# seqan/lambda

Measured on AMD Instinct MI355X. Metric: GCUPS (gapped extension, full-rectangle parity mode; pass-1 cells per second of whole step) searchp BLOSUM62, higher is better.
Workload: dtype f16x2 (exact small integers) + int32

## Files before the change

### lambda_amd/csrc/lx_ckpt.hip

```cpp
#include <hip/hip_runtime.h>

#include <algorithm>
#include <cstdlib>

#include "lx_aids.h"
#include "lx_dp_common.h"

namespace lx
{

#ifndef LX_CKPT_EVERY
#define LX_CKPT_EVERY 16
#endif
constexpr int kCkptEvery = LX_CKPT_EVERY;
#ifndef LX_CKPT_UNROLL
#define LX_CKPT_UNROLL 4
#endif
#define LX_CKPT_PRAGMA(x) _Pragma(#x)
#define LX_CKPT_UNROLL_N(n) LX_CKPT_PRAGMA(unroll n)
#define LX_CKPT_UNROLL_PRAGMA LX_CKPT_UNROLL_N(LX_CKPT_UNROLL)
#ifndef LX_BT_TILE_AT
#define LX_BT_TILE_AT 40
#endif
#ifndef LX_BT_WAVES
#define LX_BT_WAVES 2
#endif
#ifndef LX_BT_HOPS
#define LX_BT_HOPS 2
#endif
#ifndef LX_BT_REFILL_AT
#define LX_BT_REFILL_AT 12
#endif
#ifndef LX_CKPT_FWD_WAVES
#define LX_CKPT_FWD_WAVES 4
#endif

template <int G>
__host__ __device__ constexpr uint32_t bnd_quad_index(uint32_t quad, uint32_t g)
{
    return quad * G + g;
}
#ifndef LX_CKPT_ROWCK_LANE_MAJOR
#define LX_CKPT_ROWCK_LANE_MAJOR 1
#endif
template <int G, int kCkDw>
__host__ __device__ constexpr uint32_t rowck_quad_index(uint32_t m, uint32_t g, uint32_t x)
{
    return LX_CKPT_ROWCK_LANE_MAJOR ? (m * G + g) * (kCkDw / 4) + x : (m * (kCkDw / 4) + x) * G + g;
}
template <int G, int C>
struct CkptLayout
{
    static constexpr int kCkDw = (C + 3) / 4 * 4;
    __host__ __device__ static constexpr uint64_t bnd_dwords(uint32_t steps_cap) { return (uint64_t)steps_cap * G; }
    __host__ __device__ static constexpr uint64_t slot_dwords(uint32_t steps_cap)
    {
        return bnd_dwords(steps_cap) + (uint64_t)(steps_cap / kCkptEvery) * G * kCkDw;
    }
};

__device__ __forceinline__ uint32_t pack16(int lo, int hi)
{
    return ((uint32_t)lo & 0xffffu) | ((uint32_t)hi << 16);
}

template <int G, int C, bool KNOWN, bool MULTI>
__global__ __launch_bounds__(64, (KNOWN ? LX_CKPT_FWD_WAVES : 3)) void ckpt_forward_kernel(TraceParams p)
{
    using Geo = ScoreGeo<G, C>;
    using Lay = CkptLayout<G, C>;
    extern __shared__ uint32_t lds[];

    int const  lane     = threadIdx.x;
    int const  grp      = lane / G;
    int const  g        = lane % G;
    bool const is_first = (g == 0);
    bool const is_last  = (g == G - 1);

    uint64_t const e     = (uint64_t)blockIdx.x * Geo::kGroups + grp;
    uint64_t       limit = p.n;
    if (p.count_ptr)
    {
        uint64_t const total = *p.count_ptr;
        limit = total > p.chunk_start ? min(p.n, total - p.chunk_start) : 0;
        if ((uint64_t)blockIdx.x * Geo::kGroups >= limit)
            return;
    }
    bool active = e < limit;
    if (active && p.src && p.src[e] == 0xffffffffu)
        active = false;
    bool in_list = e < limit;
    if constexpr (!KNOWN)
    {
        if (p.fixup)
        {
            bool const mine = in_list && p.score_out[e] == -1;
            if (__ballot(mine) == 0)
                return;
            active  = active && mine;
            in_list = mine;
        }
    }

    ScoringDev const * __restrict__ sc = p.sc;
    int const      ge    = sc->ge;
    int const      g2    = sc->g2;
    int const      nrows = p.nrows;
    uint32_t const padt  = (uint32_t)(nrows - 1);

    int             lq = 0, ls = 0;
    uint8_t const * q = p.q_res;
    uint8_t const * s = p.s_res;
    uint64_t        q_off = 0;
    if (e < limit)
    {
        Extension const x = p.ext[e];
        lq    = (int)x.q_len;
        q_off = x.q_off;
        q += x.q_off;
        if (active)
        {
            ls = (int)x.s_len;
            if (ls != 0)
                s += x.s_off;
        }
    }
    int const share  = p.shared_profile > 1 ? min(p.shared_profile, Geo::kGroups) : 1;
    int const leader = (grp / share) * share * G;
    if (share > 1)
    {
        uint32_t const qlo = (uint32_t)__shfl((int)(uint32_t)q_off, leader), qhi = (uint32_t)__shfl((int)(q_off >> 32), leader);
        int const      l0  = __shfl(lq, leader);
        bool const     lead_in = __shfl(in_list ? 1 : 0, leader) != 0;
        if (in_list && lead_in && (q_off != (((uint64_t)qhi << 32) | qlo) || lq != l0))
            atomicExch(p.err, 2);
    }

    int       ls_max    = ls;
    int       npanels   = (lq + Geo::kPanel - 1) / Geo::kPanel;
    int const my_panels = npanels;
#pragma unroll
    for (int off = 32; off >= 1; off >>= 1)
    {
        ls_max = max(ls_max, __shfl_xor(ls_max, off));
        if constexpr (MULTI)
            npanels = max(npanels, __shfl_xor(npanels, off));
    }
    ls_max = __builtin_amdgcn_readfirstlane(ls_max);
    if constexpr (MULTI)
        npanels = max(1, __builtin_amdgcn_readfirstlane(npanels));
    else
        npanels = 1;

    bool bad = false;
    if (active && (lq > (MULTI ? (int)p.panels_cap : 1) * Geo::kPanel || (uint32_t)((ls + G - 1 + 3) & ~3) > p.steps_cap || ls > 65535))
    {
        bad = true;
        atomicExch(p.err, 3);
    }
    if (bad)
        ls = 0;

    int32_t * carry = nullptr;
    if constexpr (MULTI)
    {
        if (npanels > 1)
        {
            uint32_t base = 0;
            int      ok   = 1;
            if (is_first && my_panels > 1 && active && !bad)
            {
                base = atomicAdd(p.ws_top, (uint32_t)ls);
                if (base + (uint32_t)ls > p.ws_cap)
                {
                    ok = 0;
                    atomicExch(p.err, 1);
                }
            }
#pragma unroll
            for (int off = G / 2; off >= 1; off >>= 1)
            {
                base = max(base, (uint32_t)__shfl_xor((int)base, off));
                ok   = min(ok, __shfl_xor(ok, off));
            }
            if (my_panels > 1 && ok)
                carry = p.ws + 2ull * base;
            else if (my_panels > 1)
            {
                bad = true;
                ls  = 0;
            }
        }
    }

    int const      slot_dw     = (grp / share) * (nrows * Geo::kRowDw);
    uint32_t const row_base_dw = (uint32_t)(slot_dw + g);
    int const      steps       = (ls_max + G - 1 + 3) & ~3;
    uint32_t const lsc         = (uint32_t)max(ls, 1) - 1u;

    uint32_t * slot = p.trace + e * p.slot_stride;
    uint32_t   ovf_tag = 0;
    if constexpr (!KNOWN)
    {
        if (p.fixup && p.ovf_count)
        {
            uint32_t idx = 0;
            if (is_first && active && !bad)
                idx = atomicAdd(p.ovf_count, 1u);
            idx = (uint32_t)__shfl((int)idx, grp * G);
            if (active && !bad && idx >= p.ovf_cap)
            {
                bad = true;
                ls  = 0;
                atomicExch(p.err, 4);
            }
            ovf_tag = idx + 1;
            slot    = p.ovf + (uint64_t)(bad ? 0 : idx) * p.ovf_stride;
        }
    }
    int tgt = 0;
    if constexpr (KNOWN)
        tgt = active ? p.score_in[e] : 0;
    int kcol = 0x7fffffff, krow = 0;
    int run_best = 0, run_strip = 0, run_row = 0, run_tie = 0;
    uint64_t const panel_dw = Lay::slot_dwords(p.steps_cap);

    for (int panel = 0; panel < npanels; ++panel)
    {
    bool const    in_panel = panel < my_panels;
    bool const    store_ok = active && !bad && in_panel;
    uint32_t * const pslot = slot + (uint64_t)(MULTI ? panel : 0) * panel_dw;
    uint4 * const rowck    = reinterpret_cast<uint4 *>(pslot + Lay::bnd_dwords(p.steps_cap));
    int lbest = 0, lrow = 0, ltie = 0;
    bool use_carry_in = false, do_carry_out = false;
    if constexpr (MULTI)
    {
        use_carry_in = is_first && panel > 0 && in_panel && carry != nullptr;
        do_carry_out = is_last && panel + 1 < my_panels && carry != nullptr;
    }

    int const col0 = (MULTI ? panel * Geo::kPanel : 0) + g * C;
    build_profile<G, C>(lds, slot_dw, g, q, lq, col0, sc->mat_adj, nrows, grp % share == 0);
    __builtin_amdgcn_fence(__ATOMIC_RELEASE, "wavefront");
    __builtin_amdgcn_wave_barrier();

    int z = ge * g;
    int Hrow[C], F0[C];
#pragma unroll
    for (int c = 0; c < C; ++c)
    {
        Hrow[c] = z + ge;
        F0[c]   = z;
    }
    int diag0 = z + ge;
    int sendH = z + ge;
    int sendE = kNegInf;
    int g2v = g2, gev = ge;
    LX_OPAQUE(g2v);
    LX_OPAQUE(gev);

    uint32_t * const stage = lds + ((Geo::kGroups + share - 1) / share) * (nrows * Geo::kRowDw) + lane * 4;
    uint4 * const    bnd   = reinterpret_cast<uint4 *>(pslot);

    auto step = [&](int k, uint32_t t)
    {
        int const        i    = k - g;
        uint32_t const * prow = lds + (row_base_dw + t * (uint32_t)Geo::kRowDw);
        uint32_t         pw[Geo::kD];
#pragma unroll
        for (int d = 0; d < Geo::kD; ++d)
            pw[d] = prow[d * G];

        int bndH = z, bndE = kNegInf;
        if constexpr (MULTI)
        {
            if (use_carry_in && (unsigned)i < (unsigned)ls)
            {
                bndH = carry[2 * i];
                bndE = carry[2 * i + 1];
            }
        }
        int const recvH = shift_from_left<G>(sendH, bndH, is_first);
        int       Ecur  = shift_from_left<G>(sendE, bndE, is_first);
        int       dg    = diag0;
        diag0           = recvH;

        int const zn     = z - gev;
        int       rowmax = z;
        int       h      = 0;
#pragma unroll
        for (int c = 0; c < C; ++c)
        {
            int const sub = (int)(int8_t)(pw[c >> 2] >> (8 * (c & 3)));
            int const tt  = dg + sub;
            dg            = Hrow[c];
            h             = max3i(tt, Ecur, F0[c]);
            LX_OPAQUE(h);
            int const A   = h + g2v;
            F0[c]         = max3i(F0[c], A, zn);
            LX_OPAQUE(F0[c]);
            Ecur          = max(Ecur, A) + gev;
            if (c & 1)
                rowmax = max3i(rowmax, Hrow[c - 1], h);
            else if (c == C - 1)
                rowmax = max(rowmax, h);
            Hrow[c] = h;
        }
        if constexpr (KNOWN)
        {
            if (tgt > 0 && rowmax == tgt + z && (unsigned)i < (unsigned)ls)
            {
#pragma unroll
                for (int c = C - 1; c >= 0; --c)
                    if (Hrow[c] == rowmax && col0 + c < kcol)
                    {
                        kcol = col0 + c;
                        krow = i;
                    }
            }
        }
        else
        {
            int const  cand = rowmax - z;
            bool const gt   = cand > lbest;
            ltie            = gt ? 0 : (ltie | (cand == lbest ? 1 : 0));
            lrow            = gt ? i : lrow;
            lbest           = max(lbest, cand);
        }
        sendH = h;
        sendE = Ecur;
        if constexpr (MULTI)
        {
            if (do_carry_out && (unsigned)i < (unsigned)ls)
            {
                carry[2 * i]     = sendH;
                carry[2 * i + 1] = sendE;
            }
        }
        stage[k & 3] = pack16(h - z, max(Ecur - z, -32768));
        z            = zn;
    };
    auto checkpoint = [&](int k)
    {
        if (!store_ok)
            return;
#pragma unroll
        for (int x = 0; x < Lay::kCkDw / 4; ++x)
        {
            uint32_t w[4];
#pragma unroll
            for (int b = 0; b < 4; ++b)
            {
                int const c = 4 * x + b;
                w[b]        = c < C ? pack16(Hrow[c < C ? c : 0] - (z + gev), F0[c < C ? c : 0] - z) : 0u;
            }
            rowck[rowck_quad_index<G, Lay::kCkDw>((uint32_t)(k / kCkptEvery), (uint32_t)g, (uint32_t)x)] = make_uint4(w[0], w[1], w[2], w[3]);
        }
    };

    auto fetch_checked = [&](int k0, uint32_t (&t)[4])
    {
#pragma unroll
        for (int u = 0; u < 4; ++u)
        {
            uint32_t const i   = (uint32_t)(k0 + u - g);
            uint32_t const idx = min(i, lsc);
            t[u]               = s[idx];
        }
    };
    auto mask_checked = [&](int k0, uint32_t (&t)[4])
    {
#pragma unroll
        for (int u = 0; u < 4; ++u)
        {
            uint32_t const i = (uint32_t)(k0 + u - g);
            t[u]             = (i < (uint32_t)ls) ? (t[u] & (kAlph - 1)) : padt;
        }
    };

    uint32_t tn[4];
    fetch_checked(0, tn);
    for (int k0 = 0; k0 < steps; k0 += 4)
    {
        uint32_t tc[4] = {tn[0], tn[1], tn[2], tn[3]};
        mask_checked(k0, tc);
        fetch_checked(k0 + 4, tn);
        uint32_t const tcp = tc[0] | (tc[1] << 8) | (tc[2] << 16) | (tc[3] << 24);
LX_CKPT_UNROLL_PRAGMA
        for (int u = 0; u < 4; ++u)
            step(k0 + u, (tcp >> (8 * u)) & 0xffu);
        if (store_ok)
            bnd[bnd_quad_index<G>((uint32_t)k0 / 4, (uint32_t)g)] = *reinterpret_cast<uint4 const *>(stage);
        if (((k0 + 3) % kCkptEvery) == kCkptEvery - 1)
            checkpoint(k0 + 3);
    }

    if constexpr (!KNOWN)
    {
        int gbest = lbest, gstrip = g, grow = lrow, gtie = ltie;
#pragma unroll
        for (int off = 1; off < G; off <<= 1)
        {
            int const  ob = __shfl_xor(gbest, off), os = __shfl_xor(gstrip, off), orow = __shfl_xor(grow, off), ot = __shfl_xor(gtie, off);
            bool const take = ob > gbest || (ob == gbest && os < gstrip);
            gbest  = take ? ob : gbest;
            gstrip = take ? os : gstrip;
            grow   = take ? orow : grow;
            gtie   = take ? ot : gtie;
        }
        bool const take = gbest > run_best;
        run_best  = take ? gbest : run_best;
        run_strip = take ? (MULTI ? panel * G : 0) + gstrip : run_strip;
        run_row   = take ? grow : run_row;
        run_tie   = take ? gtie : run_tie;
    }
    if constexpr (MULTI)
    {
        if (npanels > 1)
        {
            __builtin_amdgcn_fence(__ATOMIC_RELEASE, "workgroup");
            __builtin_amdgcn_s_waitcnt(0);
            __builtin_amdgcn_fence(__ATOMIC_ACQUIRE, "workgroup");
        }
    }
    __builtin_amdgcn_wave_barrier();
    }

    if constexpr (KNOWN)
    {
#pragma unroll
        for (int off = 1; off < G; off <<= 1)
        {
            int const  oc = __shfl_xor(kcol, off), orow = __shfl_xor(krow, off);
            bool const take = oc < kcol;
            kcol = take ? oc : kcol;
            krow = take ? orow : krow;
        }
        if (in_list && is_first)
        {
            EndCell ec{};
            if (bad || (tgt > 0 && kcol == 0x7fffffff))
                ec.score = -1;
            else if (tgt > 0)
            {
                ec.score = tgt;
                ec.q_end = kcol + 1;
                ec.s_end = krow + 1;
            }
            p.ends[e] = ec;
        }
    }
    else
    {
        int const gbest = run_best, gstrip = run_strip, grow = run_row, gtie = run_tie;
        if (in_list && is_first)
        {
            EndCell ec{};
            if (bad)
                ec.score = -1;
            else if (active && gbest > 0)
            {
                ec.score = gbest;
                ec.q_end = -(gstrip + 1);
                ec.s_end = grow + 1;
                ec.flags = (gtie ? kEndAmbiguous : 0) | (int32_t)(ovf_tag << kEndOverflowShift);
            }
            p.ends[e] = ec;
            if (p.score_out)
                p.score_out[e] = bad ? -1 : (active ? gbest : 0);
        }
    }
}

template <int G, int C>
__global__ __launch_bounds__(64, LX_BT_WAVES) void ckpt_backtrace_kernel(TraceParams p)
{
    using Lay               = CkptLayout<G, C>;
    using L16               = Ckpt16Layout<G, C>;
    constexpr int kNibDw    = (C + 7) / 8;
    constexpr int kFar      = -(1 << 28);
    static_assert(kCkptEvery == 16, "the diagonal shortcut reads at most 16 residues per sequence");
    __shared__ int8_t   smat4[kAlph * kAlph];
    __shared__ int8_t   smat1n[kAlph * kAlph];
    __shared__ uint32_t tiles[kCkptEvery * kNibDw * 64];
    for (int x = threadIdx.x; x < kAlph * kAlph; x += blockDim.x)
    {
        int const v = p.sc->mat[x];
        smat4[x]    = (int8_t)((v < -32 || v > 31) ? -125 : 4 * v + 3);
        smat1n[x]   = (int8_t)(x == kAlph * kAlph - 1 ? 0 : min(-v, 127));
    }
    __syncthreads();
    uint32_t const lane  = threadIdx.x;
    uint64_t       limit = p.n;
    if (p.count_ptr)
    {
        uint64_t const total = *p.count_ptr;
        limit = total > p.chunk_start ? min(p.n, total - p.chunk_start) : 0;
    }
    int const ge = p.sc->ge, g2 = p.sc->g2;
    int const ge4 = 4 * p.sc->ge, go4 = 4 * p.sc->go;
    uint64_t panel_dw = Lay::slot_dwords(p.steps_cap), panel16_dw = L16::slot_dwords(p.steps_cap), bnd_dw = Lay::bnd_dwords(p.steps_cap);

    bool             have = false, blocked = false, done = false, need_col = false, scan = false, c16 = false;
    uint64_t         po = 0;
    uint64_t         pos = 0;
    EndCell          ec{};
    uint32_t const * slot = nullptr;
    uint32_t         oct_mul = G, ck_mul = G * (L16::kCkDw / 4);
    uint64_t         ck16_off = 0;
    uint8_t const *  q = nullptr, * s = nullptr;
    uint8_t *        ops_al = nullptr;
    uint32_t         cap = 0, a0 = 0, apos = 0, acc = 0, n = 0;
    int              lq = 0, ls = 0;
    int              i = 0, j = 0, end_i = 0, end_j = 0;
    int              res_col = C, res_row = 0x7fffffff;
    int              nar_cw = C, nar_j0 = 0x7fffffff, nar_st0 = 0x7fffffff;
    auto locate = [&](int aj, int & st, int & j0, int & cw)
    {
        if (aj >= nar_j0)
        {
            int const jl = aj - nar_j0;
            int const gl = nar_cw == (3 * C + 3) / 4 ? jl / ((3 * C + 3) / 4) : nar_cw == (C + 1) / 2 ? jl / ((C + 1) / 2) : jl / ((C + 3) / 4);
            st = nar_st0 + gl;
            j0 = nar_j0 + gl * nar_cw;
            cw = nar_cw;
        }
        else
        {
            st = aj / C;
            j0 = st * C;
            cw = C;
        }
    };
    int              mode = 0;
    int              left = 0;
    int32_t          nm = 0, nx = 0, np = 0, go = 0, gx = 0;
    bool const       rle_mode = p.rle != nullptr;
    uint32_t         run_op = 3, run_len = 0, ncodes = 0;

    auto dec = [](uint32_t bits16) -> int { return (int)(int16_t)bits16; };
    auto expand = [](uint32_t code16) -> uint32_t
    {
        uint32_t const H = code16 & 0x7ffu;
        return H | ((H - (code16 >> 11)) << 16);
    };
    auto bnd_of = [&](uint32_t pn) { return reinterpret_cast<uint4 const *>(slot + (uint64_t)pn * (c16 ? panel16_dw : panel_dw)); };
    auto rowck_of = [&](uint32_t pn)
    {
        return reinterpret_cast<uint4 const *>(slot + (c16 ? (uint64_t)pn * panel16_dw + ck16_off
                                                           : (uint64_t)pn * panel_dw + bnd_dw));
    };
    auto oct16_index = [&](uint32_t o, uint32_t g_) -> uint32_t { return o * oct_mul + g_; };
    auto ck16_index  = [&](uint32_t m_, uint32_t g_, uint32_t x_) -> uint32_t { return m_ * ck_mul + g_ * (L16::kCkDw / 4) + x_; };
    auto rowck_word = [&](uint32_t m, uint32_t st, uint32_t c) -> uint32_t
    {
        if (c16)
            return expand(reinterpret_cast<uint16_t const *>(rowck_of(st / G) + ck16_index(m, st % G, c / 8))[c % 8]);
        return reinterpret_cast<uint32_t const *>(rowck_of(st / G) + rowck_quad_index<G, Lay::kCkDw>(m, st % G, c / 4))[c % 4];
    };
    auto bnd_word_of = [&](uint32_t st, uint32_t k) -> uint32_t
    {
        if (c16)
            return expand(reinterpret_cast<uint16_t const *>(bnd_of(st / G) + oct16_index(k / 8, st % G))[k & 7]);
        return reinterpret_cast<uint32_t const *>(bnd_of(st / G) + bnd_quad_index<G>(k / 4, st % G))[k & 3];
    };
    auto put_byte = [&](uint32_t byte)
    {
        acc |= byte << (8 * (apos & 3));
        if ((apos & 3) == 0)
        {
            if (apos + 3 <= a0 + cap - 1)
                *reinterpret_cast<uint32_t *>(ops_al + apos) = acc;
            else
                for (uint32_t b = 0; b < 4 && apos + b <= a0 + cap - 1; ++b)
                    ops_al[apos + b] = (uint8_t)(acc >> (8 * b));
            acc = 0;
        }
        --apos;
    };
    auto emit = [&](uint32_t op)
    {
        if (rle_mode)
        {
            uint32_t const oc = op == (uint32_t)'M' ? 0u : (op == (uint32_t)'D' ? 1u : 2u);
            if (oc != run_op || run_len == 64)
            {
                if (run_op != 3)
                {
                    put_byte((run_op << 6) | (run_len - 1));
                    ++ncodes;
                }
                run_op  = oc;
                run_len = 0;
            }
            ++run_len;
        }
        else
            put_byte(op);
        ++n;
    };

    auto begin_extension = [&](uint64_t e)
    {
        uint64_t oi = e;
        if (p.src)
        {
            uint32_t const sidx = p.src[e];
            if (sidx == 0xffffffffu)
                return;
            oi = sidx;
        }
        pos                = e;
        po                 = p.out_by_pos ? e : oi;
        uint64_t const  se = p.slot_by_src ? oi : e;
        ec                 = p.ends[se];
        Extension const x  = p.ext[e];
        if (ec.score <= 0)
        {
            Hsp out{};
            out.score     = ec.score < 0 ? -1 : 0;
            p.out_hsp[po] = out;
            return;
        }
        c16                = (ec.flags & kEndCompact) != 0;
        uint32_t const ovf = (uint32_t)ec.flags >> kEndOverflowShift;
        slot               = ovf ? p.ovf + (uint64_t)(ovf - 1) * p.ovf_stride : p.trace + se * p.slot_stride;
        uint32_t steps_e   = p.steps_cap;
        if (p.wf_tab && !ovf)
        {
            WfSlots const  t      = p.wf_tab[se / 16];
            uint64_t const stride = (uint64_t)t.panels_cap * (c16 ? L16::slot_dwords(t.steps_cap) : Lay::slot_dwords(t.steps_cap));
            slot                  = ((p.split_n != 0 && se >= p.split_n) ? p.trace2 : p.trace) + t.off_dw + (se % 16) * stride;
            steps_e               = t.steps_cap;
        }
        panel_dw           = Lay::slot_dwords(steps_e);
        panel16_dw         = L16::slot_dwords(steps_e);
        bnd_dw             = Lay::bnd_dwords(steps_e);
        oct_mul            = G;
        ck_mul             = G * (L16::kCkDw / 4);
        ck16_off           = L16::bnd_dwords(steps_e);
        if (!ovf && (ec.flags & kEndWaveSlots))
        {
            constexpr uint32_t kW = 128 / G;
            uint64_t const     w  = se % kW;
            slot     = p.trace + (se - w) * p.slot_stride + w * (G * 4);
            oct_mul  = kW * G;
            ck_mul   = kW * G * (L16::kCkDw / 4);
            ck16_off = (uint64_t)kW * L16::bnd_dwords(steps_e) - w * (G * 4) + w * (G * L16::kCkDw);
        }
        q                  = p.q_res + x.q_off;
        s                  = p.s_res + x.s_off;
        uint8_t * const ops = p.out_ops + (p.ops_off ? p.ops_off[po] : po * p.ops_stride);
        cap                = x.q_len + x.s_len;
        lq                 = (int)x.q_len;
        ls                 = (int)x.s_len;
        i                  = ec.s_end - 1;
        j                  = ec.q_end - 1;
        {
            int const code = (ec.flags >> kEndNarrowShift) & 3;
            int const last = max(1, (lq + G * C - 1) / (G * C)) - 1;
            nar_cw  = narrow_strip_cols(C, code);
            nar_j0  = code ? last * (G * C) : 0x7fffffff;
            nar_st0 = code ? last * G : 0x7fffffff;
        }
        need_col = ec.q_end < 0;
        if (need_col)
        {
            int const st = -ec.q_end - 1;
            j = st >= nar_st0 ? nar_j0 + (st - nar_st0) * nar_cw + (nar_cw - 1) : st * C + (C - 1);
            scan = (ec.flags & kEndAmbiguous) != 0;
            if (scan)
            {
                int const gl = st % G;
                i            = min(((i + gl) / kCkptEvery) * kCkptEvery - gl + kCkptEvery - 1, ls - 1);
            }
        }
        end_i = i;
        end_j = j;
        res_col = C;
        res_row = 0x7fffffff;
        mode = 0;
        left = ec.score;
        n    = 0;
        nm = nx = np = go = gx = 0;
        a0     = (uint32_t)(reinterpret_cast<uintptr_t>(ops) & 3);
        ops_al = ops - a0;
        apos   = a0 + cap - 1;
        acc    = 0;
        run_op  = 3;
        run_len = 0;
        ncodes  = 0;
        have    = true;
        done    = false;
        blocked = false;
    };

    auto close_ops = [&]()
    {
        if (mode != 0)
            go += 1;
        if (rle_mode && run_op != 3)
        {
            put_byte((run_op << 6) | (run_len - 1));
            ++ncodes;
        }
        if ((apos & 3) != 3)
            for (uint32_t b = (apos & 3) + 1; b < 4 && (apos & ~3u) + b <= a0 + cap - 1; ++b)
                ops_al[(apos & ~3u) + b] = (uint8_t)(acc >> (8 * b));
    };
    auto finish_extension = [&](uint64_t at)
    {
        if (rle_mode && ec.score >= 0)
        {
            if (at + ncodes > p.rle_cap)
            {
                atomicExch(p.err, 5);
                ec.score = -1;
            }
            else
            {
                uint8_t const * const src = ops_al + apos + 1;
                uint8_t * const       dst = p.rle + at;
                for (uint32_t k = 0; k < ncodes; ++k)
                    dst[k] = src[k];
            }
        }
        Hsp out{};
        if (ec.score < 0)
            out.score = -1;
        else
        {
            out.score              = ec.score;
            out.q_begin            = j + 1;
            out.q_end              = end_j + 1;
            out.s_begin            = i + 1;
            out.s_end              = end_i + 1;
            out.n_ops              = (int32_t)n;
            out.num_matches        = nm;
            out.num_mismatches     = nx;
            out.num_positives      = np;
            out.num_gap_opens      = go;
            out.num_gap_extensions = gx;
            out.ops_shift          = rle_mode ? (int32_t)(uint32_t)at : (int32_t)(cap - n);
        }
        p.out_hsp[po] = out;
        if (rle_mode && p.rle_len)
            p.rle_len[pos] = ec.score > 0 ? ncodes : 0u;
        have          = false;
    };


    auto load_diagonal = [&](int ci, int cj, int k, uint32_t (&qw)[4], uint32_t (&sw)[4])
    {
#pragma unroll
        for (int d = 0; d < 4; ++d)
        {
            qw[d] = *reinterpret_cast<unaligned_u32 const *>(q + (cj - k + 1) + 4 * d);
            sw[d] = *reinterpret_cast<unaligned_u32 const *>(s + (ci - k + 1) + 4 * d);
        }
    };
    auto take_diagonal = [&](int k, int Hb, bool verify, uint32_t (&qw)[4], uint32_t (&sw)[4]) -> bool
    {
#pragma unroll
        for (int d = 0; d < 4; ++d)
        {
            int const      nb  = k - 4 * d;
            uint32_t const pad = nb >= 4 ? 0u : (nb <= 0 ? 0x1f1f1f1fu : (0x1f1f1f1fu << (8 * nb)));
            qw[d]              = (qw[d] & 0x1f1f1f1fu) | pad;
            sw[d]              = (sw[d] & 0x1f1f1f1fu) | pad;
        }
        int      P = 0, cnt = 0;
        uint32_t posbits = 0;
        int32_t  tmb = 0;
        bool const bs = p.bs_match_rule != 0;
#pragma unroll
        for (int u = kCkptEvery - 1; u >= 0; --u)
        {
            int const      d   = u >> 2, b = u & 3;
            uint32_t const idx = (((qw[d] >> (8 * b)) & 0x1fu) << 5) | ((sw[d] >> (8 * b)) & 0x1fu);
            int const      nv  = (int)smat1n[idx];
            bool const     take = P < left;
            int const      nve = take ? nv : 0;
            cnt += take ? 1 : 0;
            P -= nve;
            posbits = __builtin_amdgcn_alignbit(posbits, (uint32_t)nve, 31);
            if (bs)
                tmb += (take && nv == (int)smat1n[(idx >> 5) * (kAlph + 1)]) ? 1 : 0;
        }
        int const beyond = left > 0 ? kCkptEvery - k : 0;
        cnt -= beyond;
        tmb -= bs ? beyond : 0;
        int const  L       = left - P;
        bool const stopped = cnt < k;
        if (!(stopped ? (L == 0) : (!verify || L == Hb)))
            return false;
        int32_t tm = tmb;
        if (!bs)
        {
            int const lo = k - cnt;
#pragma unroll
            for (int d = 0; d < 4; ++d)
            {
                uint32_t const x   = qw[d] ^ sw[d];
                uint32_t const nz  = (x + 0x7f7f7f7fu) & 0x80808080u;
                int const      b0  = max(lo - 4 * d, 0), b1 = min(k - 4 * d, 4);
                uint32_t const msk = b1 > b0 ? ((b1 >= 4 ? 0xffffffffu : ((1u << (8 * b1)) - 1u)) & ~((1u << (8 * b0)) - 1u)) : 0u;
                tm += __popc(~nz & 0x80808080u & msk);
            }
        }
        left = L;
        nm += tm;
        nx += cnt - tm;
        np += __popc(posbits);
        if (rle_mode)
        {
            int left_m = cnt;
            while (left_m > 0)
            {
                if (run_op != 0 || run_len == 64)
                {
                    if (run_op != 3)
                    {
                        put_byte((run_op << 6) | (run_len - 1));
                        ++ncodes;
                    }
                    run_op  = 0;
                    run_len = 0;
                }
                int const take = min(left_m, 64 - (int)run_len);
                run_len += (uint32_t)take;
                left_m -= take;
            }
        }
        else if (cnt > 0)
        {
            uint32_t const hi = apos, lo = apos + 1 - (uint32_t)cnt, Dtop = hi & ~3u, Dlow = lo & ~3u;
#pragma unroll
            for (int sl = 0; sl < 5; ++sl)
            {
                uint32_t const D = Dtop - 4u * sl;
                if (Dtop >= 4u * sl && D >= Dlow)
                {
                    uint32_t const b0  = lo > D ? lo - D : 0, b1 = sl == 0 ? hi - D : 3u;
                    uint32_t const msk = (b1 >= 3 ? 0xffffffffu : ((1u << (8 * (b1 + 1))) - 1u)) & ~((1u << (8 * b0)) - 1u);
                    uint32_t const val = (sl == 0 ? acc : 0u) | (0x4d4d4d4du & msk);
                    if (lo <= D)
                    {
                        if (sl != 0 || D + 3 <= a0 + cap - 1)
                            *reinterpret_cast<uint32_t *>(ops_al + D) = val;
                        else
                            for (uint32_t bb = 0; bb < 4 && D + bb <= a0 + cap - 1; ++bb)
                                ops_al[D + bb] = (uint8_t)(val >> (8 * bb));
                        acc = 0;
                    }
                    else
                        acc = val;
                }
            }
            apos -= (uint32_t)cnt;
        }
        n += (uint32_t)cnt;
        i -= cnt;
        j -= cnt;
        done = stopped;
        return true;
    };

    bool queue_empty = false;
    int const tile_at = p.bt_tile_at > 0 ? p.bt_tile_at : LX_BT_TILE_AT, refill_at = p.bt_refill_at > 0 ? p.bt_refill_at : LX_BT_REFILL_AT;
    for (;;)
    {
        bool fin       = have && (done || i < 0 || j < 0 || n >= cap);
        bool can       = have && !fin && !blocked && !need_col && mode == 0;
        bool tile_need = have && !fin && !can;
        int  n_can = __popcll(__ballot(can)), n_tile = __popcll(__ballot(tile_need));
        int const n_idle = 64 - n_can - n_tile;
        bool run_tile = n_can == 0 || n_tile >= tile_at;
        if (n_idle > 0 && (run_tile || n_idle >= refill_at))
        {
            if (fin)
                close_ops();
            uint64_t at = 0;
            if (rle_mode)
            {
                uint32_t const mine = fin ? ncodes : 0u;
                uint32_t       incl = mine;
#pragma unroll
                for (int off = 1; off < 64; off <<= 1)
                {
                    uint32_t const up = (uint32_t)__shfl_up((int)incl, off);
                    if ((int)lane >= off)
                        incl += up;
                }
                uint32_t const     total = (uint32_t)__shfl((int)incl, 63);
                unsigned long long base  = 0;
                if (lane == 63 && total != 0)
                    base = atomicAdd(p.rle_top, (unsigned long long)total);
                base = ((unsigned long long)(uint32_t)__shfl((int)(base >> 32), 63) << 32) | (uint32_t)__shfl((int)(uint32_t)base, 63);
                at   = base + incl - mine;
            }
            if (fin)
                finish_extension(at);
            if (!queue_empty)
            {
                uint64_t const want = __ballot(!have);
                if (want != 0)
                {
                    uint32_t  base   = 0;
                    int const leader = __ffsll((unsigned long long)want) - 1;
                    if ((int)lane == leader)
                        base = atomicAdd(p.work_counter, (uint32_t)__popcll(want));
                    base = (uint32_t)__shfl((int)base, leader);
                    if ((uint64_t)base + (uint32_t)__popcll(want) >= limit)
                        queue_empty = true;
                    if (!have)
                    {
                        uint64_t const e = (uint64_t)base + (uint32_t)__popcll(want & ((1ull << lane) - 1ull));
                        if (e < limit)
                            begin_extension(e);
                    }
                }
            }
            fin       = have && (done || i < 0 || j < 0 || n >= cap);
            can       = have && !fin && !blocked && !need_col && mode == 0;
            tile_need = have && !fin && !can;
            n_can     = __popcll(__ballot(can));
            n_tile    = __popcll(__ballot(tile_need));
            if (n_can == 0 && n_tile == 0)
            {
                if (__ballot(have) == 0 && queue_empty)
                    break;
                if (__ballot(have) == 0)
                    continue;
            }
            run_tile = n_can == 0 || n_tile >= tile_at;
        }

        if (!run_tile)
        {
            if (can)
            {
                int      hk[LX_BT_HOPS];
                uint32_t hw[LX_BT_HOPS], hqw[LX_BT_HOPS][4], hsw[LX_BT_HOPS][4];
                int      ci = i, cj = j;
#pragma unroll
                for (int h = 0; h < LX_BT_HOPS; ++h)
                {
                    bool const on = ci >= 0 && cj >= 0;
                    int const ai = max(ci, 0), aj = max(cj, 0);
                    int st, j0, cw;
                    locate(aj, st, j0, cw);
                    int const c  = aj - j0;
                    int const gl = st % G;
                    int const m  = (ai + gl) / kCkptEvery;
                    int const r_base = m * kCkptEvery - gl;
                    int const kt = ai - r_base + 1, kl = c + 1;
                    int const k  = min(min(kt, kl), ai + 1);
                    int const bi = ai - k, bj = aj - k;
                    hk[h] = on ? k : 0;
                    hw[h] = 0;
                    if (on && bi >= 0 && bj >= 0)
                        hw[h] = (kl <= kt) ? bnd_word_of((uint32_t)(st - 1), (uint32_t)(bi + (st - 1) % G))
                                           : rowck_word((uint32_t)(m - 1), (uint32_t)st, (uint32_t)(bj - j0));
                    load_diagonal(ai, aj, k, hqw[h], hsw[h]);
                    ci -= k;
                    cj -= k;
                }
#pragma unroll
                for (int h = 0; h < LX_BT_HOPS; ++h)
                    if (hk[h] > 0 && !blocked && !done)
                        if (!take_diagonal(hk[h], dec(hw[h] & 0xffffu), true, hqw[h], hsw[h]))
                            blocked = true;
            }
            continue;
        }

        if (tile_need)
        {
        int st, j0, cw;
        locate(j, st, j0, cw);
        int const pn = st / G, gl = st % G;
        int const m  = (i + gl) / kCkptEvery;
        int const k_base = m * kCkptEvery;
        int const r_base = k_base - gl;
        uint4 const * const rowck = rowck_of((uint32_t)pn);

        int Hp[C], F[C];
        if (m == 0)
        {
#pragma unroll
            for (int c = 0; c < C; ++c)
            {
                Hp[c] = 0;
                F[c]  = 2;
            }
        }
        else
        {
            uint32_t      w[Lay::kCkDw];
            if (c16)
            {
#pragma unroll
                for (int xq = 0; xq < L16::kCkDw / 4; ++xq)
                {
                    uint4 const    v    = rowck[ck16_index((uint32_t)(m - 1), (uint32_t)gl, (uint32_t)xq)];
                    uint32_t const d[4] = {v.x, v.y, v.z, v.w};
#pragma unroll
                    for (int b = 0; b < 4; ++b)
                    {
                        int const c = 2 * (4 * xq + b);
                        if (c < Lay::kCkDw)
                            w[c] = expand(d[b] & 0xffffu);
                        if (c + 1 < Lay::kCkDw)
                            w[c + 1] = expand(d[b] >> 16);
                    }
                }
            }
            else
            {
#pragma unroll
                for (int xq = 0; xq < Lay::kCkDw / 4; ++xq)
                {
                    uint4 const v = rowck[rowck_quad_index<G, Lay::kCkDw>((uint32_t)(m - 1), (uint32_t)gl, (uint32_t)xq)];
                    w[4 * xq] = v.x; w[4 * xq + 1] = v.y; w[4 * xq + 2] = v.z; w[4 * xq + 3] = v.w;
                }
            }
#pragma unroll
            for (int c = 0; c < C; ++c)
            {
                Hp[c] = 4 * dec(w[c] & 0xffffu);
                F[c]  = (4 * dec(w[c] >> 16)) | 2;
            }
        }
        uint32_t qoff2[(C + 1) / 2];
        uint32_t qd[(C + 3) / 4];
        {
#pragma unroll
            for (int d = 0; d < (C + 3) / 4; ++d)
                qd[d] = *reinterpret_cast<unaligned_u32 const *>(q + j0 + 4 * d);
#pragma unroll
            for (int c = 0; c < C; ++c)
            {
                uint32_t const r = (c < cw && j0 + c < lq) ? ((qd[c >> 2] >> (8 * (c & 3))) & (kAlph - 1)) : (uint32_t)(kAlph - 1);
                qoff2[c >> 1]    = (c & 1) ? (qoff2[c >> 1] | ((r * kAlph) << 16)) : r * kAlph;
            }
        }
        bool const has_left = st > 0;
        int const  gL       = gl > 0 ? gl - 1 : G - 1;
        int const  qshift   = (gl == 0 && has_left) ? G / 4 : 0;
        uint4 const * const bndL = bnd_of((uint32_t)(gl > 0 ? pn : max(pn - 1, 0)));
        auto load_bq = [&](int qd) -> uint4
        {
            if (!has_left || qd + qshift < 0)
                return make_uint4(0, 0, 0, 0);
            if (c16)
            {
                int const   qs = qd + qshift;
                uint2 const v  = reinterpret_cast<uint2 const *>(bndL + oct16_index((uint32_t)qs / 2, (uint32_t)gL))[qs & 1];
                return make_uint4(expand(v.x & 0xffffu), expand(v.x >> 16), expand(v.y & 0xffffu), expand(v.y >> 16));
            }
            return bndL[bnd_quad_index<G>((uint32_t)(qd + qshift), (uint32_t)gL)];
        };
        int const qd0   = k_base / 4;
        uint4     qprev = load_bq(qd0 - 1), qcur = load_bq(qd0);

        uint32_t snext = *reinterpret_cast<unaligned_u32 const *>(s + max(r_base, 0));
#pragma unroll 1
        for (int t = 0; t < kCkptEvery / 4; ++t)
        {
            if (__ballot(r_base + 4 * t <= i) == 0)
                break;
            uint4 const qnext = load_bq(qd0 + t + 1);
            int const      row0 = r_base + 4 * t;
            int const      lb   = max(row0, 0);
            uint32_t const sdw  = snext;
            snext               = *reinterpret_cast<unaligned_u32 const *>(s + max(row0 + 4, 0));
            uint32_t const lw[4] = {qprev.w, qcur.x, qcur.y, qcur.z};
            uint32_t const dw[4] = {qprev.z, qprev.w, qcur.x, qcur.y};
#pragma unroll
            for (int u = 0; u < 4; ++u)
            {
                int const      row = row0 + u;
                uint32_t const tl  = row >= 0 ? (sdw >> (8 * (row - lb))) & (kAlph - 1) : (uint32_t)(kAlph - 1);
                int            E   = (has_left && row >= 0) ? ((4 * dec(lw[u] >> 16)) | 1) : (kFar | 1);
                int            Hd  = (has_left && row > 0) ? 4 * dec(dw[u] & 0xffffu) : 0;
                uint32_t       w[kNibDw];
#pragma unroll
                for (int xw = 0; xw < kNibDw; ++xw)
                    w[xw] = 0;
                int sub4[C];
#pragma unroll
                for (int c = 0; c < C; ++c)
                    sub4[c] = (int)smat4[((qoff2[c >> 1] >> (16 * (c & 1))) & 0xffffu) + tl];
#pragma unroll
                for (int c = 0; c < C; ++c)
                {
                    int const tt  = Hd + sub4[c];
                    Hd            = Hp[c];
                    int const m   = max3i(tt, E, F[c]);
                    int const H4  = m & ~3;
                    int const A   = H4 + go4;
                    int const Fr  = max3i(F[c] + ge4, A, 0);
                    int const Er  = max(E + ge4, A);
                    F[c]          = Fr | 2;
                    E             = Er | 1;
                    Hp[c]         = H4;
                    uint32_t wc   = w[c >> 3];
                    wc            = __builtin_amdgcn_alignbit((uint32_t)m, wc, 2);
                    wc            = __builtin_amdgcn_alignbit((uint32_t)(Fr | Er), wc, 2);
                    w[c >> 3]     = wc;
                }
                int const kk = 4 * t + u;
                w[kNibDw - 1] |= tl;
#pragma unroll
                for (int xw = 0; xw < kNibDw; ++xw)
                    tiles[(kk * kNibDw + xw) * 64 + lane] = w[xw];
                if (need_col && row <= i && row >= 0 && row < ls)
                {
                    int const tgt4 = 4 * ec.score;
                    int       kmax = 0;
#pragma unroll
                    for (int c = 0; c < C; ++c)
                        kmax = max(kmax, ((Hp[c] - tgt4) << 5) + (C - c));
                    int const  cmin  = C - kmax;
                    bool const lower = kmax > 0 && cmin < res_col;
                    res_col          = lower ? cmin : res_col;
                    res_row          = lower ? row : res_row;
                }
            }
            qprev = qcur;
            qcur  = qnext;
        }

        bool walk_ok = true;
        if (scan && r_base + kCkptEvery < ls)
        {
            i       = min(r_base + 2 * kCkptEvery - 1, ls - 1);
            walk_ok = false;
        }
        else if (need_col)
        {
            need_col = false;
            scan     = false;
            walk_ok  = false;
            if (res_col >= C)
            {
                done     = true;
                left     = -1;
                ec.score = -1;
            }
            else
            {
                i     = res_row;
                j     = j0 + res_col;
                end_i = i;
                end_j = j;
            }
        }
        static_assert(32 - 4 * (C - 8 * (kNibDw - 1)) >= 5, "the last nibble word needs 5 spare bits for the subject letter");
        bool passed = false;
        if (walk_ok && mode == 0 && i >= 0 && j >= j0 && i >= r_base)
        {
            int const kk = i - r_base, c = j - j0;
            int const kmax = min(min(kk, c), i) + 1;
            uint32_t  nd = 0;
#pragma unroll
            for (int t = 0; t < kCkptEvery; ++t)
            {
                int const      rr   = max(kk - t, 0), cc = max(c - t, 0);
                int const      xw   = cc >> 3;
                uint32_t const word = tiles[(rr * kNibDw + xw) * 64 + lane];
                int const      sh   = (xw == kNibDw - 1 ? 32 - 4 * (C - 8 * (kNibDw - 1)) : 0) + 4 * (cc & 7);
                nd |= (((word >> sh) & 3u) != 3u) ? (1u << t) : 0u;
            }
            nd |= ~0u << kmax;
            int const d = __ffs((int)nd) - 1;
            if (d > 0)
            {
                uint32_t qw[4], sw[4];
                load_diagonal(i, j, d, qw, sw);
                (void)take_diagonal(d, 0, false, qw, sw);
            }
        }
        while (walk_ok && !done && i >= 0 && j >= j0 && i >= r_base && n < cap && !(passed && mode == 0))
        {
            int const      kk   = i - r_base, c = j - j0;
            int const      xw   = c >> 3;
            int const      cnt  = (xw == kNibDw - 1) ? (C - 8 * xw) : 8;
            uint32_t const word = tiles[(kk * kNibDw + xw) * 64 + lane];
            uint32_t const last = tiles[(kk * kNibDw + (kNibDw - 1)) * 64 + lane];
            uint32_t const nib  = (word >> (32 - 4 * cnt + 4 * (c & 7))) & 15u;
            bool const     in_v = mode == 1, in_h = mode == 2;
            bool const     cont = (in_v && (nib & 8u)) || (in_h && (nib & 4u));
            bool const     leave = (in_v || in_h) && !cont;
            go += leave ? 1 : 0;
            left -= leave ? g2 : 0;
            if (!cont && left <= 0)
            {
                done = true;
                break;
            }
            uint32_t const code = nib & 3u;
            bool const     diag = !cont && code == 3, vert = cont ? in_v : code == 2;
            uint32_t qsel = qd[0];
#pragma unroll
            for (int d = 1; d < (C + 3) / 4; ++d)
                qsel = ((c >> 2) == d) ? qd[d] : qsel;
            uint32_t const c0 = (qsel >> (8 * (c & 3))) & (kAlph - 1), c1 = last & (kAlph - 1);
            int const      sm = (int)smat4[c0 * kAlph + c1];
            int const      v  = (sm - 3) >> 2;
            bool const     isMatch = p.bs_match_rule ? (sm == (int)smat4[c0 * kAlph + c0]) : (c0 == c1);
            nm += (diag && isMatch) ? 1 : 0;
            nx += (diag && !isMatch) ? 1 : 0;
            np += (diag && v > 0) ? 1 : 0;
            gx += cont ? 1 : 0;
            left -= diag ? v : ge;
            mode = diag ? 0 : (vert ? 1 : 2);
            passed = passed || !diag;
            emit(diag ? (uint32_t)'M' : (vert ? (uint32_t)'D' : (uint32_t)'I'));
            i -= (diag || vert) ? 1 : 0;
            j -= (diag || !vert) ? 1 : 0;
        }
        blocked = false;
        }
    }
}


uint64_t ckpt_slot_dwords(int cfg, uint32_t steps_cap)
{
    return cfg == 2   ? CkptLayout<16, 13>::slot_dwords(steps_cap)
           : cfg == 3 ? CkptLayout<8, 13>::slot_dwords(steps_cap)
           : cfg == 4 ? CkptLayout<8, 25>::slot_dwords(steps_cap)
           : cfg == 5 ? CkptLayout<8, 11>::slot_dwords(steps_cap)
                      : CkptLayout<8, 19>::slot_dwords(steps_cap);
}

uint64_t ckpt16_slot_dwords(int cfg, uint32_t steps_cap)
{
    return cfg == 2   ? Ckpt16Layout<16, 13>::slot_dwords(steps_cap)
           : cfg == 3 ? Ckpt16Layout<8, 13>::slot_dwords(steps_cap)
           : cfg == 4 ? Ckpt16Layout<8, 25>::slot_dwords(steps_cap)
           : cfg == 5 ? Ckpt16Layout<8, 11>::slot_dwords(steps_cap)
                      : Ckpt16Layout<8, 19>::slot_dwords(steps_cap);
}

template <int G, int C>
static hipError_t launch_ckpt_forward_cfg(TraceParams const & p, hipStream_t stream)
{
    using Geo = ScoreGeo<G, C>;
    uint64_t const blocks = (p.n + Geo::kGroups - 1) / Geo::kGroups;
    if (blocks > 0x7fffffffull || (!p.score_in && !p.score_out) || p.steps_cap % kCkptEvery != 0)
        return hipErrorInvalidValue;
    int const    share = p.shared_profile > 1 ? std::min(p.shared_profile, Geo::kGroups) : 1;
    int const    slots = (Geo::kGroups + share - 1) / share;
    size_t const lds   = ((size_t)slots * (size_t)p.nrows * Geo::kRowDw + 64 * 4) * sizeof(uint32_t);
    bool const multi = p.panels_cap > 1;
    if (lds > 64 * 1024)
    {
        hipError_t const ea = multi ? hipFuncSetAttribute(reinterpret_cast<void const *>(&ckpt_forward_kernel<G, C, false, true>),
                                                          hipFuncAttributeMaxDynamicSharedMemorySize, (int)lds)
                                    : hipFuncSetAttribute(reinterpret_cast<void const *>(&ckpt_forward_kernel<G, C, false, false>),
                                                          hipFuncAttributeMaxDynamicSharedMemorySize, (int)lds);
        if (ea != hipSuccess || p.score_in)
            return ea != hipSuccess ? ea : hipErrorInvalidValue;
    }
    if (p.score_in && multi)
        hipLaunchKernelGGL((ckpt_forward_kernel<G, C, true, true>), dim3((unsigned)blocks), dim3(64), lds, stream, p);
    else if (p.score_in)
        hipLaunchKernelGGL((ckpt_forward_kernel<G, C, true, false>), dim3((unsigned)blocks), dim3(64), lds, stream, p);
    else if (multi)
        hipLaunchKernelGGL((ckpt_forward_kernel<G, C, false, true>), dim3((unsigned)blocks), dim3(64), lds, stream, p);
    else
        hipLaunchKernelGGL((ckpt_forward_kernel<G, C, false, false>), dim3((unsigned)blocks), dim3(64), lds, stream, p);
    return hipGetLastError();
}

hipError_t launch_ckpt_forward(TraceParams const & p, hipStream_t stream)
{
    if (p.n == 0)
        return hipSuccess;
    return p.cfg == 2   ? launch_ckpt_forward_cfg<16, 13>(p, stream)
           : p.cfg == 3 ? launch_ckpt_forward_cfg<8, 13>(p, stream)
           : p.cfg == 4 ? launch_ckpt_forward_cfg<8, 25>(p, stream)
           : p.cfg == 5 ? launch_ckpt_forward_cfg<8, 11>(p, stream)
                        : launch_ckpt_forward_cfg<8, 19>(p, stream);
}

static int backtrace_resident_waves()
{
    static int const v = []()
    {
        int dev = 0, cus = 256;
        if (hipGetDevice(&dev) == hipSuccess)
            (void)hipDeviceGetAttribute(&cus, hipDeviceAttributeMultiprocessorCount, dev);
        int const per_cu = 4 * LX_BT_WAVES;
        return std::max(1, cus) * per_cu;
    }();
    return v;
}

hipError_t launch_ckpt_backtrace(TraceParams const & p_in, hipStream_t stream)
{
    if (p_in.n == 0)
        return hipSuccess;
    if (!p_in.work_counter)
        return hipErrorInvalidValue;
    TraceParams p = p_in;
    {
        p.bt_tile_at   = dev_aids().bt_tile_at;
        p.bt_refill_at = dev_aids().bt_refill_at;
    }
    uint64_t const b2 = std::min<uint64_t>((p.n + 63) / 64, (uint64_t)backtrace_resident_waves());
    hipError_t e = hipMemsetAsync(p.work_counter, 0, sizeof(uint32_t), stream);
    if (e != hipSuccess)
        return e;
    if (p.cfg == 2)
        hipLaunchKernelGGL((ckpt_backtrace_kernel<16, 13>), dim3((unsigned)b2), dim3(64), 0, stream, p);
    else if (p.cfg == 3)
        hipLaunchKernelGGL((ckpt_backtrace_kernel<8, 13>), dim3((unsigned)b2), dim3(64), 0, stream, p);
    else if (p.cfg == 4)
        hipLaunchKernelGGL((ckpt_backtrace_kernel<8, 25>), dim3((unsigned)b2), dim3(64), 0, stream, p);
    else if (p.cfg == 5)
        hipLaunchKernelGGL((ckpt_backtrace_kernel<8, 11>), dim3((unsigned)b2), dim3(64), 0, stream, p);
    else
        hipLaunchKernelGGL((ckpt_backtrace_kernel<8, 19>), dim3((unsigned)b2), dim3(64), 0, stream, p);
    return hipGetLastError();
}

}
```

Baseline: 5546.

## Park divergent backtrace lanes in an LDS pool to raise per-phase lane occupancy

Adds a per-wave shared-memory pool where lanes whose extension is in the wrong phase (shortcut vs tile) serialise their full traceback state and give up their slot. Pooled records are later swapped back into lanes that are empty or in the other phase, so each shortcut or tile pass runs with more active lanes. The refill threshold is also raised and refill now triggers whenever no lane can take the shortcut path. This costs extra LDS for up to 32 ten-quad records per wave, which may reduce occupancy, plus register pressure and ballot overhead for packing and unpacking state. An optional compile-time counter probe is included.

```diff
diff --git a/lambda_amd/csrc/lx_ckpt.hip b/lambda_amd/csrc/lx_ckpt.hip
--- a/lambda_amd/csrc/lx_ckpt.hip
+++ b/lambda_amd/csrc/lx_ckpt.hip
@@ -1,6 +1,7 @@
 #include <hip/hip_runtime.h>
 
 #include <algorithm>
+#include <cstdio>
 #include <cstdlib>
 
 #include "lx_aids.h"
@@ -29,10 +30,16 @@
 #define LX_BT_HOPS 2
 #endif
 #ifndef LX_BT_REFILL_AT
-#define LX_BT_REFILL_AT 12
+#define LX_BT_REFILL_AT 24
+#endif
+#ifndef LX_BT_POOL
+#define LX_BT_POOL 32
 #endif
 #ifndef LX_CKPT_FWD_WAVES
 #define LX_CKPT_FWD_WAVES 4
+#endif
+#ifdef LX_BT_COUNT
+__device__ unsigned long long lx_bt_counts[5];
 #endif
 
 template <int G>
@@ -483,6 +490,11 @@
     __shared__ int8_t   smat4[kAlph * kAlph];
     __shared__ int8_t   smat1n[kAlph * kAlph];
     __shared__ uint32_t tiles[kCkptEvery * kNibDw * 64];
+    constexpr int kRecQ  = 10;
+    constexpr int kLdsWg = 20 * 1024 - (int)sizeof(uint32_t) * kCkptEvery * kNibDw * 64 - 2 * kAlph * kAlph;
+    constexpr int kPool  = LX_BT_POOL < kLdsWg / (16 * kRecQ) ? LX_BT_POOL : kLdsWg / (16 * kRecQ);
+    static_assert(kPool >= 0 && kPool <= 64, "pool masks are 64 bits wide");
+    __shared__ uint4 pool[kRecQ][kPool > 0 ? kPool : 1];
     for (int x = threadIdx.x; x < kAlph * kAlph; x += blockDim.x)
     {
         int const v = p.sc->mat[x];
@@ -749,6 +761,94 @@
         have          = false;
     };
 
+    auto park = [&](uint32_t e)
+    {
+        uint32_t const flags = (blocked ? 1u : 0u) | (done ? 2u : 0u) | (need_col ? 4u : 0u) | (scan ? 8u : 0u) | (c16 ? 16u : 0u) |
+                               ((uint32_t)mode << 5) | (run_op << 7) | (run_len << 9) | (a0 << 16) | ((uint32_t)nar_cw << 18) |
+                               ((uint32_t)res_col << 24);
+        uint64_t const sp = reinterpret_cast<uintptr_t>(slot), qp = reinterpret_cast<uintptr_t>(q), spp = reinterpret_cast<uintptr_t>(s),
+                       op = reinterpret_cast<uintptr_t>(ops_al);
+        pool[0][e] = make_uint4(flags, (uint32_t)pos, (uint32_t)po, (uint32_t)ec.score);
+        pool[1][e] = make_uint4((uint32_t)sp, (uint32_t)(sp >> 32), oct_mul, ck_mul);
+        pool[2][e] = make_uint4((uint32_t)ck16_off, (uint32_t)panel_dw, (uint32_t)panel16_dw, (uint32_t)bnd_dw);
+        pool[3][e] = make_uint4((uint32_t)qp, (uint32_t)(qp >> 32), (uint32_t)spp, (uint32_t)(spp >> 32));
+        pool[4][e] = make_uint4((uint32_t)op, (uint32_t)(op >> 32), cap, apos);
+        pool[5][e] = make_uint4(acc, n, (uint32_t)lq, (uint32_t)ls);
+        pool[6][e] = make_uint4((uint32_t)i, (uint32_t)j, (uint32_t)end_i, (uint32_t)end_j);
+        pool[7][e] = make_uint4((uint32_t)res_row, (uint32_t)nar_j0, (uint32_t)nar_st0, (uint32_t)left);
+        pool[8][e] = make_uint4((uint32_t)nm, (uint32_t)nx, (uint32_t)np, (uint32_t)go);
+        pool[9][e] = make_uint4((uint32_t)gx, ncodes, 0u, 0u);
+    };
+    auto unpark = [&](uint4 const (&r)[kRecQ])
+    {
+        uint32_t const flags = r[0].x;
+        blocked  = (flags & 1u) != 0;
+        done     = (flags & 2u) != 0;
+        need_col = (flags & 4u) != 0;
+        scan     = (flags & 8u) != 0;
+        c16      = (flags & 16u) != 0;
+        mode     = (int)((flags >> 5) & 3u);
+        run_op   = (flags >> 7) & 3u;
+        run_len  = (flags >> 9) & 127u;
+        a0       = (flags >> 16) & 3u;
+        nar_cw   = (int)((flags >> 18) & 63u);
+        res_col  = (int)((flags >> 24) & 63u);
+        pos      = r[0].y;
+        po       = r[0].z;
+        ec.score = (int32_t)r[0].w;
+        slot     = reinterpret_cast<uint32_t const *>(((uint64_t)r[1].y << 32) | r[1].x);
+        oct_mul  = r[1].z;
+        ck_mul   = r[1].w;
+        ck16_off   = r[2].x;
+        panel_dw   = r[2].y;
+        panel16_dw = r[2].z;
+        bnd_dw     = r[2].w;
+        q      = reinterpret_cast<uint8_t const *>(((uint64_t)r[3].y << 32) | r[3].x);
+        s      = reinterpret_cast<uint8_t const *>(((uint64_t)r[3].w << 32) | r[3].z);
+        ops_al = reinterpret_cast<uint8_t *>(((uint64_t)r[4].y << 32) | r[4].x);
+        cap    = r[4].z;
+        apos   = r[4].w;
+        acc    = r[5].x;
+        n      = r[5].y;
+        lq     = (int)r[5].z;
+        ls     = (int)r[5].w;
+        i      = (int)r[6].x;
+        j      = (int)r[6].y;
+        end_i  = (int)r[6].z;
+        end_j  = (int)r[6].w;
+        res_row = (int)r[7].x;
+        nar_j0  = (int)r[7].y;
+        nar_st0 = (int)r[7].z;
+        left    = (int)r[7].w;
+        nm      = (int32_t)r[8].x;
+        nx      = (int32_t)r[8].y;
+        np      = (int32_t)r[8].z;
+        go      = (int32_t)r[8].w;
+        gx      = (int32_t)r[9].x;
+        ncodes  = r[9].y;
+        have    = true;
+    };
+    auto nth_bit = [](uint64_t m, uint32_t r) -> uint32_t
+    {
+        uint32_t at = 0;
+#pragma unroll
+        for (int w = 32; w >= 1; w >>= 1)
+        {
+            uint32_t const lo = (uint32_t)__popcll(m & ((1ull << w) - 1ull));
+            if (r >= lo)
+            {
+                r -= lo;
+                m >>= w;
+                at += (uint32_t)w;
+            }
+        }
+        return at;
+    };
+    auto low_bits = [&](uint64_t m, uint32_t r) -> uint64_t
+    {
+        return r >= (uint32_t)__popcll(m) ? m : (m & ((1ull << nth_bit(m, r)) - 1ull));
+    };
+
 
     auto load_diagonal = [&](int ci, int cj, int k, uint32_t (&qw)[4], uint32_t (&sw)[4])
     {
@@ -868,6 +968,11 @@
 
     bool queue_empty = false;
     int const tile_at = p.bt_tile_at > 0 ? p.bt_tile_at : LX_BT_TILE_AT, refill_at = p.bt_refill_at > 0 ? p.bt_refill_at : LX_BT_REFILL_AT;
+#ifdef LX_BT_COUNT
+    uint32_t cnt_sc = 0, cnt_sc_lanes = 0, cnt_tile = 0, cnt_tile_lanes = 0;
+#endif
+    uint64_t pool_used = 0, pool_tile = 0;
+    uint64_t const lanes_below = (1ull << lane) - 1ull;
     for (;;)
     {
         bool fin       = have && (done || i < 0 || j < 0 || n >= cap);
@@ -875,8 +980,9 @@
         bool tile_need = have && !fin && !can;
         int  n_can = __popcll(__ballot(can)), n_tile = __popcll(__ballot(tile_need));
         int const n_idle = 64 - n_can - n_tile;
-        bool run_tile = n_can == 0 || n_tile >= tile_at;
-        if (n_idle > 0 && (run_tile || n_idle >= refill_at))
+        int  p_tile = __popcll(pool_tile), p_can = __popcll(pool_used) - p_tile;
+        bool run_tile = n_can + p_can == 0 || n_tile + p_tile >= tile_at;
+        if (n_idle > 0 && (run_tile || n_idle >= refill_at || n_can == 0))
         {
             if (fin)
                 close_ops();
@@ -903,6 +1009,25 @@
                 finish_extension(at);
             if (!queue_empty)
             {
+                if constexpr (kPool > 0)
+                {
+                    bool const     out = have && !(run_tile ? tile_need : can);
+                    uint64_t const mo  = __ballot(out);
+                    uint64_t const fr  = ~pool_used & (kPool == 64 ? ~0ull : ((1ull << kPool) - 1ull));
+                    uint32_t const npk = min((uint32_t)__popcll(mo), (uint32_t)__popcll(fr));
+                    if (npk > 0)
+                    {
+                        uint32_t const rank = (uint32_t)__popcll(mo & lanes_below);
+                        if (out && rank < npk)
+                        {
+                            park(nth_bit(fr, rank));
+                            have = false;
+                        }
+                        uint64_t const got = low_bits(fr, npk);
+                        pool_used |= got;
+                        pool_tile |= run_tile ? 0ull : got;
+                    }
+                }
                 uint64_t const want = __ballot(!have);
                 if (want != 0)
                 {
@@ -926,15 +1051,69 @@
             tile_need = have && !fin && !can;
             n_can     = __popcll(__ballot(can));
             n_tile    = __popcll(__ballot(tile_need));
-            if (n_can == 0 && n_tile == 0)
+            if (n_can == 0 && n_tile == 0 && pool_used == 0)
             {
                 if (__ballot(have) == 0 && queue_empty)
+                {
+#ifdef LX_BT_COUNT
+                    if (lane == 0)
+                    {
+                        atomicAdd(&lx_bt_counts[0], (unsigned long long)cnt_sc);
+                        atomicAdd(&lx_bt_counts[1], (unsigned long long)cnt_sc_lanes);
+                        atomicAdd(&lx_bt_counts[2], (unsigned long long)cnt_tile);
+                        atomicAdd(&lx_bt_counts[3], (unsigned long long)cnt_tile_lanes);
+                        atomicAdd(&lx_bt_counts[4], 1ull);
+                    }
+#endif
                     break;
+                }
                 if (__ballot(have) == 0)
                     continue;
             }
-            run_tile = n_can == 0 || n_tile >= tile_at;
-        }
+            p_tile   = __popcll(pool_tile);
+            p_can    = __popcll(pool_used) - p_tile;
+            run_tile = n_can + p_can == 0 || n_tile + p_tile >= tile_at;
+        }
+        if constexpr (kPool > 0)
+        {
+            uint64_t const px = run_tile ? pool_tile : (pool_used & ~pool_tile);
+            if (px != 0)
+            {
+                bool const     empty = !have, other = have && !fin && !(run_tile ? tile_need : can);
+                uint64_t const me = __ballot(empty), mo = __ballot(other);
+                uint32_t const ne = (uint32_t)__popcll(me);
+                uint32_t const ns = min((uint32_t)__popcll(px), ne + (uint32_t)__popcll(mo));
+                if (ns > 0)
+                {
+                    uint32_t const rank = empty ? (uint32_t)__popcll(me & lanes_below) : (other ? ne + (uint32_t)__popcll(mo & lanes_below) : 64u);
+                    if (rank < ns)
+                    {
+                        uint32_t const e = nth_bit(px, rank);
+                        uint4          r[kRecQ];
+#pragma unroll
+                        for (int f = 0; f < kRecQ; ++f)
+                            r[f] = pool[f][e];
+                        if (other)
+                            park(e);
+                        unpark(r);
+                    }
+                    uint64_t const taken = low_bits(px, ns), freed = low_bits(px, min(ne, ns));
+                    pool_used &= ~freed;
+                    pool_tile = (pool_tile & ~freed) ^ (taken & ~freed);
+                    fin       = have && (done || i < 0 || j < 0 || n >= cap);
+                    can       = have && !fin && !blocked && !need_col && mode == 0;
+                    tile_need = have && !fin && !can;
+                    n_can     = __popcll(__ballot(can));
+                    n_tile    = __popcll(__ballot(tile_need));
+                }
+            }
+        }
+#ifdef LX_BT_COUNT
+        cnt_sc += run_tile ? 0u : 1u;
+        cnt_sc_lanes += run_tile ? 0u : (uint32_t)n_can;
+        cnt_tile += run_tile ? 1u : 0u;
+        cnt_tile_lanes += run_tile ? (uint32_t)n_tile : 0u;
+#endif
 
         if (!run_tile)
         {
@@ -1325,6 +1504,24 @@
         hipLaunchKernelGGL((ckpt_backtrace_kernel<8, 11>), dim3((unsigned)b2), dim3(64), 0, stream, p);
     else
         hipLaunchKernelGGL((ckpt_backtrace_kernel<8, 19>), dim3((unsigned)b2), dim3(64), 0, stream, p);
+#ifdef LX_BT_COUNT
+    {
+        unsigned long long c[5] = {};
+        e = hipGetLastError();
+        if (e == hipSuccess)
+            e = hipStreamSynchronize(stream);
+        if (e == hipSuccess)
+            e = hipMemcpyFromSymbol(c, HIP_SYMBOL(lx_bt_counts), sizeof(c));
+        unsigned long long const z[5] = {};
+        if (e == hipSuccess)
+            e = hipMemcpyToSymbol(HIP_SYMBOL(lx_bt_counts), z, sizeof(z));
+        if (e != hipSuccess)
+            return e;
+        fprintf(stderr, "LX_BT_COUNT cfg %d n %llu waves %llu: shortcut passes %llu, lanes/pass %.2f; tile phases %llu, lanes/phase %.2f\n",
+                p.cfg, (unsigned long long)p.n, c[4], c[0], c[0] ? (double)c[1] / (double)c[0] : 0.0, c[2],
+                c[2] ? (double)c[3] / (double)c[2] : 0.0);
+    }
+#endif
     return hipGetLastError();
 }
 
```

Result: faster. 5674, median of 6 (+2.3%).
